# aleju/cat-generator

Measured on AMD Instinct MI355X. Metric: images/sec per G+D step, G32up-c 32x32 RGB bs=128 per GPU, higher is better.
Workload: dtype f32

## Files before the change

cat-generator_amd/csrc/common.h:

```cpp
#pragma once
#include <hip/hip_runtime.h>
#include <algorithm>
#include <stdint.h>
#include <stdio.h>
#include <string.h>
#include "../../include/catgan.h"

namespace cg {

char* err_buf();
int fail(const char* fmt, ...);

inline hipStream_t S(void* s) { return reinterpret_cast<hipStream_t>(s); }

#define CG_HIP(call)                                                              \
    do {                                                                          \
        hipError_t e__ = (call);                                                  \
        if (e__ != hipSuccess)                                                    \
            return cg::fail("%s:%d %s -> %s", __FILE__, __LINE__, #call,          \
                            hipGetErrorString(e__));                              \
    } while (0)

#define CG_LAUNCH_CHECK()                                                         \
    do {                                                                          \
        hipError_t e__ = hipGetLastError();                                       \
        if (e__ != hipSuccess)                                                    \
            return cg::fail("%s:%d kernel launch -> %s", __FILE__, __LINE__,      \
                            hipGetErrorString(e__));                              \
    } while (0)

#define CG_REQUIRE(cond, ...)                                                     \
    do {                                                                          \
        if (!(cond)) return cg::fail(__VA_ARGS__);                                \
    } while (0)

constexpr int kNumCU = 256;

#ifndef CG_TIMING_PROBE
#define CG_TIMING_PROBE 0
#endif
#define CG_PROBE_HALF(fam, T) (((CG_TIMING_PROBE) & (fam)) ? ((T) + 1) / 2 : (T))
constexpr int kEwWgsPerCU = 4, kColReduceWgsPerCU = 1;

enum Opt {
    OPT_SKINNY, OPT_GEMM_BK32, OPT_WINO_BK, OPT_NN_TILE, OPT_TN_TILE, OPT_NN_SPLITS, OPT_TN_SPLITS,
    OPT_XCD_SWIZZLE, OPT_NN_GLDS, OPT_TN_GLDS, OPT_WINO_GLDS, OPT_PAD_SKIP, OPT_WINO3, OPT_WINO_DGRAD_FUSE, OPT_WINO_DGRAD_FUSE_LAUNCHES,
    OPT_WINO3_LAUNCHES, OPT_PACK_WIDE, OPT_SAMPLER_ATOMIC_LAUNCHES, OPT_COUNT
};
long opt(Opt o);
void opt_count(Opt o);

static inline int cdiv(long a, long b) { return (int)((a + b - 1) / b); }

constexpr size_t kColScratchBytes = 8u << 20;
void* col_scratch(hipStream_t stream);
hipStream_t queue_stream(hipStream_t ref, int cls, int slot);
int queue_class(hipStream_t ref, hipStream_t s);

constexpr int MAXG = 4;
constexpr int kMaxStridedGroups = 36;
template <typename T>
__device__ __forceinline__ T sel4(int i, T a, T b, T c, T d) { return i == 0 ? a : (i == 1 ? b : (i == 2 ? c : d)); }
__device__ __forceinline__ float4 ld4(const float* p) { return *reinterpret_cast<const float4*>(p); }
__device__ __forceinline__ float f4c(const float4& v, int i) { return i == 0 ? v.x : (i == 1 ? v.y : (i == 2 ? v.z : v.w)); }
template <typename T>
static inline void set4(T& p0, T& p1, T& p2, T& p3, const T* src, int n) {
    T* const dst[MAXG] = {&p0, &p1, &p2, &p3};
    for (int i = 0; i < MAXG; ++i) *dst[i] = (src && i < n) ? src[i] : nullptr;
}
__device__ __host__ __forceinline__ int phase_map(int a, int d, int pad) { return ((a + d - pad) >> 1) - ((a - pad) >> 1); }
static inline int phase_kp(int k, int pad) { return phase_map(0, k - 1, pad) + 1; }

struct WgradParts {
    const float* part;
    const float* bias_part;
    float* const* gw;
    float* const* gb;
    long gws;
    int ngroups, S, Cin, Cout, kH, kW, pad, ups;
    float scale;
};
int wgrad_finish(hipStream_t st, const WgradParts& w, bool defer);
void wgrad_discard_all();

constexpr int kSkinnyWgradBlocks = 512;
bool skinny_ok(int ngroups, int Cin, int Cout, int kH, int kW, int padH, int padW, int ups);
size_t skinny_wgrad_ws_bytes(int Cin, int Cout);
void skinny_valu_forward(hipStream_t st, const float* x, const float* w, const float* bias, float* y, int N, int H, int W, int Cin, int Cout);
void skinny_valu_wgrad(hipStream_t st, const float* x, const float* dy, float* part, float* bias_part, int N, int H, int W, int Cin, int Cout,
                       int blocks, long ppb);
bool skinny_mfma_ok(int Cin, int Cout, int H, int W);
int skinny_mfma_forward(hipStream_t st, const float* x, const float* w, const float* bias, float* y, int N, int H, int W, int Cin, int Cout);
int skinny_mfma_wgrad(hipStream_t st, const float* x, const float* dy, float* part, float* bias_part, int N, int H, int W, int Cin, int Cout,
                      int max_blocks);

bool head_wgrad_ok(int N, int T, int C, int Co);
int head_wgrad(hipStream_t st, const float* x, const float* dy, float* gw, float* gb, int N, int T, int C, int Co, float scale);
constexpr int kWino3UOffset = 9 * 64 * 64, kWino3UFloats = 16 * 64 * 64;
static inline bool wino3_layer(int Cout, int Cin, int kH, int kW) { return Cout == 64 && Cin == 64 && kH == 3 && kW == 3; }
bool wino3_geom_ok(int ngroups, int N, int H, int W, int Cin, int Cout, int kH, int kW, int padH, int padW, int ups);
int wino3_note_pack(hipStream_t st, int n, const float* const* w, float* const* wf, float* const* wb, const int* Cout, const int* Cin,
                    const int* kH, const int* kW, const int* wb_map);
int wino3_forward(hipStream_t st, int ngroups, const float* const* x, const float* const* wpk, const float* const* bias, float* const* y,
                  int N, int H, int W);

static inline int ew_grid(long n, int per_block = 256) {
    long b = (n + per_block - 1) / per_block;
    if (b < 1) b = 1;
    const long cap = (long)kNumCU * kEwWgsPerCU;
    if (b > cap) b = cap;
    return (int)b;
}

static inline bool al16(const void* p) { return ((uintptr_t)p & 15) == 0; }
template <class... P>
static inline bool vec_ok(long n, const P*... p) { return n % 4 == 0 && (al16(p) && ...); }

constexpr int tile_of_row_c(int l) {
    return ((l < 4 || (l >= 12 && l < 16) || (l >= 20 && l < 28)) ? 0 : 16) +
           ((l < 4 || (l >= 12 && l < 16) || (l >= 20 && l < 28)) ? (l < 4 ? l : (l < 16 ? l - 8 : l - 12)) : (l < 12 ? l - 4 : (l < 20 ? l - 8 : l - 16)));
}
__device__ __forceinline__ int tile_of_row(int l) {
    const bool ga = l < 4 || (l >= 12 && l < 16) || (l >= 20 && l < 28);
    const int rank = ga ? (l < 4 ? l : (l < 16 ? l - 8 : l - 12)) : (l < 12 ? l - 4 : (l < 20 ? l - 8 : l - 16));
    return (ga ? 0 : 16) + rank;
}
__device__ __forceinline__ void wino3_pack_item(const float* __restrict__ w, float* uf, float* ub, int idx) {
    constexpr int C = 64;
    const int co = idx / C, ci = idx % C;
    const float G[4][3] = {{1.f, 0.f, 0.f}, {.5f, .5f, .5f}, {.5f, -.5f, .5f}, {0.f, 0.f, 1.f}};
// ... 233 lines not shown
```

cat-generator_amd/csrc/ops.hip:

```cpp
#include "common.h"
#include <stdarg.h>
#include <stdlib.h>
#include <algorithm>

namespace cg {
char* err_buf() {
    static thread_local char buf[512] = {0};
    return buf;
}
int fail(const char* fmt, ...) {
    va_list ap;
    va_start(ap, fmt);
    vsnprintf(err_buf(), 512, fmt, ap);
    va_end(ap);
    return 1;
}

namespace {
struct OptDef { const char* name; long dflt; };
const OptDef kOptDefs[OPT_COUNT] = {
    {"CG_SKINNY", 1}, {"CG_GEMM_BK32", 1}, {"CG_WINO_BK", 0}, {"CG_NN_TILE", 0}, {"CG_TN_TILE", 0}, {"CG_NN_SPLITS", 0}, {"CG_TN_SPLITS", 0},
    {"CG_XCD_SWIZZLE", 7}, {"CG_NN_GLDS", 1}, {"CG_TN_GLDS", 1}, {"CG_WINO_GLDS", 1}, {"CG_PAD_SKIP", 20}, {"CG_WINO3", 1},
    {"CG_WINO_DGRAD_FUSE", 1}, {"CG_WINO_DGRAD_FUSE_LAUNCHES", 0}, {"CG_WINO3_LAUNCHES", 0}, {"CG_PACK_WIDE", 1},
    {"CG_SAMPLER_ATOMIC_LAUNCHES", 0},
};
long g_opt_val[OPT_COUNT];
int g_opt_state[OPT_COUNT];
}

}
#include <chrono>
#include <mutex>
#include <unordered_map>
#include <vector>
namespace cg {
void* col_scratch(hipStream_t stream) {
    constexpr int kPool = 8, kReserve = 4;
    static std::unordered_map<hipStream_t, void*> blocks;
    static std::vector<void*> pool;
    static std::mutex mu;
    std::lock_guard<std::mutex> lk(mu);
    auto it = blocks.find(stream);
    if (it != blocks.end()) return it->second;
    hipStreamCaptureStatus st = hipStreamCaptureStatusNone;
    const bool capturing = stream && hipStreamIsCapturing(stream, &st) == hipSuccess && st != hipStreamCaptureStatusNone;
    if (capturing && pool.empty()) {
        cg::fail("column reduce: no scratch block left for a stream first used inside a graph capture (run one pass on it before cg_graph_begin)");
        return nullptr;
    }
    if (!capturing && (int)pool.size() <= kReserve) {
        char* p = nullptr;
        hipStreamCaptureMode mode = hipStreamCaptureModeRelaxed;
        (void)hipThreadExchangeStreamCaptureMode(&mode);
        const bool ok = hipMalloc((void**)&p, kColScratchBytes * kPool) == hipSuccess &&
                        hipMemsetAsync(p, 0, kColScratchBytes * kPool, stream) == hipSuccess &&
                        hipStreamSynchronize(stream) == hipSuccess;
        (void)hipThreadExchangeStreamCaptureMode(&mode);
        if (!ok) {
            (void)hipGetLastError();
            if (pool.empty()) { cg::fail("column reduce: cannot allocate %zu bytes of scratch", kColScratchBytes * kPool); return nullptr; }
        } else
            for (int i = kPool - 1; i >= 0; --i) pool.insert(pool.begin(), p + (size_t)i * kColScratchBytes);
    }
    void* blk = pool.back();
    pool.pop_back();
    blocks[stream] = blk;
    return blk;
}
namespace {
__global__ void queue_probe_spin_k(unsigned long long ticks, int* sink) {
    const unsigned long long t0 = wall_clock64();
    while (wall_clock64() - t0 < ticks) { }
    if (ticks == ~0ull) *sink = 1;
}
struct QueuePool {
    std::vector<hipStream_t> s;
    std::unordered_map<hipStream_t, std::vector<int>> cls;
    std::mutex mu;
};
QueuePool& qpool() { static QueuePool p; return p; }
constexpr int kQueuePool = 24;

double probe_pair(hipStream_t a, hipStream_t b, bool both, unsigned long long ticks) {
    (void)hipStreamSynchronize(a);
    if (both) (void)hipStreamSynchronize(b);
    const auto t0 = std::chrono::steady_clock::now();
    hipLaunchKernelGGL(queue_probe_spin_k, dim3(1), dim3(64), 0, a, ticks, (int*)nullptr);
    if (both) hipLaunchKernelGGL(queue_probe_spin_k, dim3(1), dim3(64), 0, b, ticks, (int*)nullptr);
    (void)hipStreamSynchronize(a);
    if (both) (void)hipStreamSynchronize(b);
    return std::chrono::duration<double, std::milli>(std::chrono::steady_clock::now() - t0).count();
}
bool same_queue(hipStream_t a, hipStream_t b) {
    const unsigned long long ticks = 30000;
    int votes = 0;
    for (int r = 0; r < 3; ++r) {
        const double one = probe_pair(a, a, false, ticks), two = probe_pair(a, b, true, ticks);
        if (two > 1.6 * one) ++votes;
    }
    return votes >= 2;
}
}

int queue_classify(hipStream_t ref) {
    QueuePool& p = qpool();
    hipStreamCaptureStatus st = hipStreamCaptureStatusNone;
    if (ref && hipStreamIsCapturing(ref, &st) == hipSuccess && st != hipStreamCaptureStatusNone)
// ... 642 lines not shown
    GRID_STRIDE(i, total) {
        const int c = (int)(i % C);
        long r = i / C;
        const int ox = (int)(r % Wo); r /= Wo;
        const int oy = (int)(r % Ho);
        const long n = r / Ho;
        const long b = ((n * H + 2 * oy) * W + 2 * ox) * C + c;
        const long o01 = C, o10 = (long)W * C, o11 = (long)W * C + C;
        const float v00 = x[b], v01 = x[b + o01], v10 = x[b + o10], v11 = x[b + o11];
        int arg = 0; float m = v00;
        if (v01 > m) { m = v01; arg = 1; }
        if (v10 > m) { m = v10; arg = 2; }
        if (v11 > m) { m = v11; arg = 3; }
        const float g = dy[i];
        dx[b] = arg == 0 ? g : 0.f;
        dx[b + o01] = arg == 1 ? g : 0.f;
        dx[b + o10] = arg == 2 ? g : 0.f;
        dx[b + o11] = arg == 3 ? g : 0.f;
    }
}

template <int VW, bool SPATIAL>
__global__ void mask_mul_k(const float* x, const float* mask, float* y, long n, long HWCV, int CV) {
    typedef Vec<VW> V;
    CG_GRID_STRIDE(i, n) {
        const V m = SPATIAL ? V::ldc(mask, (int)((i / HWCV) * CV + (i % CV))) : V::load(mask, i);
        V v = V::load(x, i);
#pragma unroll
        for (int k = 0; k < VW; ++k) v[k] *= m[k];
        v.store(y, i);
    }
}
using cg::u01;
__global__ void rng_bernoulli_k(float* out, long n, float keep, float value, uint64_t seed, uint64_t offset,
                                const uint64_t* base) {
    if (base) offset += *base;
    GRID_STRIDE(i, n) { out[i] = u01(seed, offset + (uint64_t)i) < keep ? value : 0.f; }
}
__global__ void rng_uniform_k(float* out, long n, float lo, float hi, uint64_t seed, uint64_t offset,
                              const uint64_t* base) {
    if (base) offset += *base;
    GRID_STRIDE(i, n) { out[i] = lo + (hi - lo) * u01(seed, offset + (uint64_t)i); }
}
__global__ void rng_randint_k(int32_t* out, long n, int32_t range, uint64_t seed, uint64_t offset, const uint64_t* base) {
    if (base) offset += *base;
    GRID_STRIDE(i, n) {
        int32_t v = (int32_t)(u01(seed, offset + (uint64_t)i) * (float)range);
        out[i] = v < range ? v : range - 1;
    }
}
__global__ void rng_bernoulli_groups_k(float* out, long n, int G, float keep, float value, uint64_t seed, uint64_t off0,
                                       uint64_t off1, uint64_t off2, uint64_t off3, const uint64_t* base) {
    const uint64_t b = base ? *base : 0ull;
    GRID_STRIDE(i, n * G) {
        const int g = (int)(i / n);
        const uint64_t off = g == 0 ? off0 : (g == 1 ? off1 : (g == 2 ? off2 : off3));
        out[i] = u01(seed, b + off + (uint64_t)(i - (long)g * n)) < keep ? value : 0.f;
    }
}
__global__ void counter_add_k(uint64_t* c, uint64_t d) { if (threadIdx.x == 0 && blockIdx.x == 0) *c += d; }

__global__ void nchw_to_nhwc_k(const float* in, float* out, int N, int C, int H, int W) {
    const long total = (long)N * C * H * W;
    GRID_STRIDE(i, total) {
        const int c = (int)(i % C);
        long r = i / C;
        const int x = (int)(r % W); r /= W;
        const int y = (int)(r % H);
        const long n = r / H;
        out[i] = in[((n * C + c) * H + y) * W + x];
    }
}
__global__ void nhwc_to_nchw_k(const float* in, float* out, int N, int C, int H, int W) {
    const long total = (long)N * C * H * W;
    GRID_STRIDE(i, total) {
        const int x = (int)(i % W);
        long r = i / W;
        const int y = (int)(r % H); r /= H;
        const int c = (int)(r % C);
        const long n = r / C;
        out[i] = in[((n * H + y) * W + x) * C + c];
    }
}
__global__ void copy_channels_k(const float* src, float* dst, long M, int Csrc, int so, int Cdst, int dof, int Cc) {
    const long total = M * Cc;
    GRID_STRIDE(i, total) {
        const int c = (int)(i % Cc);
        const long m = i / Cc;
        dst[m * Cdst + dof + c] = src[m * Csrc + so + c];
    }
}
__global__ void gather_rows_k(const float* src, const int32_t* idx, float* dst, long nrows, long rowlen) {
    const long total = nrows * rowlen;
    GRID_STRIDE(i, total) {
        const long r = i / rowlen, j = i - r * rowlen;
        dst[i] = src[(long)idx[r] * rowlen + j];
    }
}
__global__ void fill_k(float* x, float v, long n) { GRID_STRIDE(i, n) x[i] = v; }
__global__ void axpy_sign_k(float al, const float* x, float* y, long n) {
    GRID_STRIDE(i, n) {
        const float v = x[i];
        y[i] += al * (v > 0.f ? 1.f : (v < 0.f ? -1.f : 0.f));
    }
}
__global__ void scale_k(float* x, float al, long n) { GRID_STRIDE(i, n) x[i] *= al; }
__global__ void clamp_k(float* x, float lo, float hi, long n) {
    GRID_STRIDE(i, n) { x[i] = fminf(fmaxf(x[i], lo), hi); }
}
template <bool SQ>
__global__ void sumred_k(const float* x, long n, double* out) {
    __shared__ double sh[4];
    double s = 0.0;
    GRID_STRIDE(i, n) {
        const float v = x[i];
        s += SQ ? (double)v * (double)v : (double)fabsf(v);
    }
    const double t = block_sum_256(s, sh);
    if (threadIdx.x == 0) atomicAdd(out, t);
}

__global__ void affine_matrix_fwd_k(const float* params, float* T, int N, int ur, int us, int ut) {
    const int P = ur + us + 2 * ut;
    GRID_STRIDE(n, N) {
        const float* p = params + (long)n * P;
        int k = 0;
        float th = 0.f, sc = 1.f, tx = 0.f, ty = 0.f;
        if (ur) th = p[k++];
        if (us) sc = p[k++];
        if (ut) { tx = p[k]; ty = p[k + 1]; }
        const float c = cosf(th), s = sinf(th);
        float* t = T + (long)n * 6;
        t[0] = c * sc;  t[1] = -s * sc; t[2] = c * sc * tx - s * sc * ty;
        t[3] = s * sc;  t[4] = c * sc;  t[5] = s * sc * tx + c * sc * ty;
    }
}
__global__ void affine_matrix_bwd_k(const float* params, const float* gT, float* gparams, int N, int ur, int us, int ut) {
    const int P = ur + us + 2 * ut;
    GRID_STRIDE(n, N) {
        const float* p = params + (long)n * P;
        int k = 0;
        float th = 0.f, sc = 1.f, tx = 0.f, ty = 0.f;
        if (ur) th = p[k++];
        if (us) sc = p[k++];
        if (ut) { tx = p[k]; ty = p[k + 1]; }
        const float c = cosf(th), s = sinf(th);
        const float* g = gT + (long)n * 6;
        float* gp = gparams + (long)n * P;
        k = 0;
        if (ur) {
            const float d0 = -s * sc, d1 = -c * sc, d2 = -s * sc * tx - c * sc * ty;
            const float d3 = c * sc, d4 = -s * sc, d5 = c * sc * tx - s * sc * ty;
            gp[k++] = g[0] * d0 + g[1] * d1 + g[2] * d2 + g[3] * d3 + g[4] * d4 + g[5] * d5;
        }
        if (us) {
            gp[k++] = g[0] * c + g[1] * (-s) + g[2] * (c * tx - s * ty) + g[3] * s + g[4] * c + g[5] * (s * tx + c * ty);
        }
        if (ut) {
            gp[k] = g[2] * (c * sc) + g[5] * (s * sc);
            gp[k + 1] = g[2] * (-s * sc) + g[5] * (c * sc);
        }
    }
}
__global__ void affine_grid_fwd_k(const float* T, float* grid, int N, int H, int W) {
    const long total = (long)N * H * W;
    GRID_STRIDE(i, total) {
// ... 732 lines not shown
    else EW_LAUNCH(bn_bwd_k<1>, total, x, dy, gamma, save_mean, save_invstd, sums, count, total, C, dx);
    EW_LAUNCH(bn_bwd_param_k, (long)C, local_sums, C, ggamma, gbeta, scale);
    return 0;
}

int cg_upsample2x_forward(void* stream, const float* x, float* y, int N, int H, int W, int C) {
    CG_REQUIRE(x && y, "cg_upsample2x_forward: null pointer");
    const long total = (long)N * 4 * H * W * C;
    EW_LAUNCH(ups2_fwd_k, total, x, y, N, H, W, C); return 0;
}
int cg_upsample2x_backward(void* stream, const float* dy, float* dx, int N, int H, int W, int C) {
    CG_REQUIRE(dy && dx, "cg_upsample2x_backward: null pointer");
    const long total = (long)N * H * W * C;
    EW_LAUNCH(ups2_bwd_k, total, dy, dx, N, H, W, C); return 0;
}
int cg_avgpool2_forward(void* stream, const float* x, float* y, int N, int H, int W, int C) {
    CG_REQUIRE(x && y, "cg_avgpool2_forward: null pointer");
    const long total = (long)N * (H / 2) * (W / 2) * C;
    EW_LAUNCH(pool2_fwd_k<false>, total, x, y, N, H, W, C); return 0;
}
int cg_avgpool2_backward(void* stream, const float* dy, float* dx, int N, int H, int W, int C) {
    CG_REQUIRE(dy && dx, "cg_avgpool2_backward: null pointer");
    const long total = (long)N * H * W * C;
    EW_LAUNCH(avgpool2_bwd_k, total, dy, dx, N, H, W, C); return 0;
}
int cg_maxpool2_forward(void* stream, const float* x, float* y, int N, int H, int W, int C) {
    CG_REQUIRE(x && y, "cg_maxpool2_forward: null pointer");
    const long total = (long)N * (H / 2) * (W / 2) * C;
    EW_LAUNCH(pool2_fwd_k<true>, total, x, y, N, H, W, C); return 0;
}
int cg_maxpool2_backward(void* stream, const float* x, const float* dy, float* dx, int N, int H, int W, int C) {
    CG_REQUIRE(x && dy && dx, "cg_maxpool2_backward: null pointer");
    CG_REQUIRE(H % 2 == 0 && W % 2 == 0, "cg_maxpool2_backward: odd spatial size");
    const long total = (long)N * (H / 2) * (W / 2) * C;
    EW_LAUNCH(maxpool2_bwd_k, total, x, dy, dx, N, H, W, C); return 0;
}
int cg_mask_mul(void* stream, const float* x, const float* mask, float* y, int N, long HW, int C, int spatial) {
    CG_REQUIRE(x && mask && y, "cg_mask_mul: null pointer");
    const long total = (long)N * HW * C;
    const bool v4 = spatial ? cg::vec_ok(C, x, y) : cg::vec_ok(total, x, y, mask);
    if (v4 && spatial) EW_LAUNCH((mask_mul_k<4, true>), total / 4, x, mask, y, total / 4, HW * C / 4, C / 4);
    else if (v4) EW_LAUNCH((mask_mul_k<4, false>), total / 4, x, mask, y, total / 4, 0L, 0);
    else if (spatial) EW_LAUNCH((mask_mul_k<1, true>), total, x, mask, y, total, HW * C, C);
    else EW_LAUNCH((mask_mul_k<1, false>), total, x, mask, y, total, 0L, 0);
    return 0;
}
int cg_rng_bernoulli_dev(void* stream, float* out, long n, float keep_prob, float value, uint64_t seed, uint64_t offset,
                         const uint64_t* base) {
    CG_REQUIRE(out, "cg_rng_bernoulli: null pointer");
    EW_LAUNCH(rng_bernoulli_k, n, out, n, keep_prob, value, seed, offset, base); return 0;
}
int cg_rng_bernoulli_dev_grouped(void* stream, float* out, long n_per_group, int ngroups, float keep_prob, float value,
                                 uint64_t seed, uint64_t off0, uint64_t off1, uint64_t off2, uint64_t off3,
                                 const uint64_t* base) {
    CG_REQUIRE(out && ngroups >= 1 && ngroups <= 4, "cg_rng_bernoulli_dev_grouped: bad args");
    EW_LAUNCH(rng_bernoulli_groups_k, n_per_group * ngroups, out, n_per_group, ngroups, keep_prob, value, seed, off0, off1, off2,
              off3, base);
    return 0;
}
int cg_rng_uniform_dev(void* stream, float* out, long n, float lo, float hi, uint64_t seed, uint64_t offset,
                       const uint64_t* base) {
    CG_REQUIRE(out, "cg_rng_uniform: null pointer");
    EW_LAUNCH(rng_uniform_k, n, out, n, lo, hi, seed, offset, base); return 0;
}
int cg_rng_randint_dev(void* stream, int32_t* out, long n, int32_t range, uint64_t seed, uint64_t offset,
                       const uint64_t* base) {
    CG_REQUIRE(out && range > 0, "cg_rng_randint: bad args");
    EW_LAUNCH(rng_randint_k, n, out, n, range, seed, offset, base); return 0;
}
int cg_rng_bernoulli(void* stream, float* out, long n, float keep_prob, float value, uint64_t seed, uint64_t offset) {
    return cg_rng_bernoulli_dev(stream, out, n, keep_prob, value, seed, offset, nullptr);
}
int cg_rng_uniform(void* stream, float* out, long n, float lo, float hi, uint64_t seed, uint64_t offset) {
    return cg_rng_uniform_dev(stream, out, n, lo, hi, seed, offset, nullptr);
}
int cg_rng_randint(void* stream, int32_t* out, long n, int32_t range, uint64_t seed, uint64_t offset) {
    return cg_rng_randint_dev(stream, out, n, range, seed, offset, nullptr);
}
int cg_counter_add(void* stream, uint64_t* counter, uint64_t delta) {
    CG_REQUIRE(counter, "cg_counter_add: null pointer");
    hipLaunchKernelGGL(counter_add_k, dim3(1), dim3(64), 0, cg::S(stream), counter, delta);
    CG_LAUNCH_CHECK(); return 0;
}
int cg_nchw_to_nhwc(void* stream, const float* in, float* out, int N, int C, int H, int W) {
    CG_REQUIRE(in && out, "cg_nchw_to_nhwc: null pointer");
    const long total = (long)N * C * H * W;
    EW_LAUNCH(nchw_to_nhwc_k, total, in, out, N, C, H, W); return 0;
}
int cg_nhwc_to_nchw(void* stream, const float* in, float* out, int N, int C, int H, int W) {
    CG_REQUIRE(in && out, "cg_nhwc_to_nchw: null pointer");
    const long total = (long)N * C * H * W;
    EW_LAUNCH(nhwc_to_nchw_k, total, in, out, N, C, H, W); return 0;
}
int cg_copy_channels(void* stream, const float* src, float* dst, long M, int Csrc, int src_off, int Cdst, int dst_off,
                     int Ccopy) {
    CG_REQUIRE(src && dst, "cg_copy_channels: null pointer");
    CG_REQUIRE(src_off >= 0 && dst_off >= 0 && src_off + Ccopy <= Csrc && dst_off + Ccopy <= Cdst,
               "cg_copy_channels: slice out of range");
    const long total = M * Ccopy;
    EW_LAUNCH(copy_channels_k, total, src, dst, M, Csrc, src_off, Cdst, dst_off, Ccopy); return 0;
}
int cg_gather_rows(void* stream, const float* src, const int32_t* idx, float* dst, long nrows, long rowlen) {
    CG_REQUIRE(src && idx && dst, "cg_gather_rows: null pointer");
    const long total = nrows * rowlen;
    EW_LAUNCH(gather_rows_k, total, src, idx, dst, nrows, rowlen); return 0;
}
int cg_fill(void* stream, float* x, float value, long n) {
    CG_REQUIRE(x, "cg_fill: null pointer");
    EW_LAUNCH(fill_k, n, x, value, n); return 0;
}
int cg_add(void* stream, const float* a, const float* b, float* out, long n) {
    CG_REQUIRE(a && b && out, "cg_add: null pointer");
    if (cg::vec_ok(n, a, b, out)) EW_LAUNCH(add_k<4>, n / 4, a, b, out, n / 4);
    else EW_LAUNCH(add_k<1>, n, a, b, out, n);
    return 0;
}
int cg_axpy(void* stream, float alpha, const float* x, float* y, long n) {
    CG_REQUIRE(x && y, "cg_axpy: null pointer");
    if (cg::vec_ok(n, x, y)) EW_LAUNCH(axpy_k<4>, n / 4, alpha, x, y, n / 4);
    else EW_LAUNCH(axpy_k<1>, n, alpha, x, y, n);
    return 0;
}
int cg_axpy_sign(void* stream, float alpha, const float* x, float* y, long n) {
    CG_REQUIRE(x && y, "cg_axpy_sign: null pointer");
    EW_LAUNCH(axpy_sign_k, n, alpha, x, y, n); return 0;
}
int cg_scale(void* stream, float* x, float alpha, long n) {
    CG_REQUIRE(x, "cg_scale: null pointer");
    EW_LAUNCH(scale_k, n, x, alpha, n); return 0;
}
int cg_clamp(void* stream, float* x, float lo, float hi, long n) {
    CG_REQUIRE(x, "cg_clamp: null pointer");
    EW_LAUNCH(clamp_k, n, x, lo, hi, n); return 0;
}
int cg_sumsq(void* stream, const float* x, long n, double* out) {
    CG_REQUIRE(x && out, "cg_sumsq: null pointer");
    CG_HIP(hipMemsetAsync(out, 0, sizeof(double), cg::S(stream)));
    EW_LAUNCH(sumred_k<true>, n, x, n, out); return 0;
}
int cg_sumabs(void* stream, const float* x, long n, double* out) {
    CG_REQUIRE(x && out, "cg_sumabs: null pointer");
    CG_HIP(hipMemsetAsync(out, 0, sizeof(double), cg::S(stream)));
    EW_LAUNCH(sumred_k<false>, n, x, n, out); return 0;
}

int cg_affine_matrix_forward(void* stream, const float* params, float* T, int N, int use_rot, int use_scale,
                             int use_trans) {
    CG_REQUIRE(params && T, "cg_affine_matrix_forward: null pointer");
    CG_REQUIRE(use_rot || use_scale || use_trans, "cg_affine_matrix_forward: fully parametrised form not supported");
    EW_LAUNCH(affine_matrix_fwd_k, (long)N, params, T, N, use_rot ? 1 : 0, use_scale ? 1 : 0, use_trans ? 1 : 0);
    return 0;
}
int cg_affine_matrix_backward(void* stream, const float* params, const float* gT, float* gparams, int N, int use_rot,
                              int use_scale, int use_trans) {
    CG_REQUIRE(params && gT && gparams, "cg_affine_matrix_backward: null pointer");
    EW_LAUNCH(affine_matrix_bwd_k, (long)N, params, gT, gparams, N, use_rot ? 1 : 0, use_scale ? 1 : 0, use_trans ? 1 : 0);
    return 0;
}
int cg_affine_grid_forward(void* stream, const float* T, float* grid, int N, int H, int W) {
    CG_REQUIRE(T && grid, "cg_affine_grid_forward: null pointer");
    const long total = (long)N * H * W;
    EW_LAUNCH(affine_grid_fwd_k, total, T, grid, N, H, W); return 0;
}
int cg_affine_grid_backward(void* stream, const float* ggrid, float* gT, int N, int H, int W) {
    CG_REQUIRE(ggrid && gT && N > 0, "cg_affine_grid_backward: bad args");
    hipLaunchKernelGGL(affine_grid_bwd_k, dim3(N), dim3(256), 0, cg::S(stream), ggrid, gT, N, H, W);
    CG_LAUNCH_CHECK(); return 0;
}
namespace {
int sampler_forward(void* stream, const float* img, const float* grid, float* out, int N, int Nimg, int Hi, int Wi, int C, int Ho,
                    int Wo) {
    const long total = (long)N * Ho * Wo * C;
    if (cg::vec_ok(C, img, out) && (uintptr_t)grid % 8 == 0) EW_LAUNCH(bilinear_fwd_k<4>, total / 4, img, grid, out, N, Nimg, Hi, Wi, C / 4, Ho, Wo);
// ... 112 lines not shown
```

cat-generator_amd/csrc/wgrad_finish.hip:

```cpp
#include "common.h"
#include <mutex>
#include <unordered_map>
#include <vector>

namespace {

using cg::f4c;
using cg::ld4;
using cg::phase_map;
using cg::sel4;

template <bool UPS, int STEP>
__device__ __forceinline__ float fold(const float* pg, int tap, int ci, int co, int Cin, int Cout, int k, int pad, int kp, long plane, int S,
                                      long sstride, int sp0) {
    float s = 0.f;
    if (UPS) {
        const int dy = tap / k, dx = tap - dy * k;
        for (int sp = sp0; sp < S; sp += STEP)
#pragma unroll
            for (int p = 0; p < 4; ++p) {
                const int tp = phase_map(p >> 1, dy, pad) * kp + phase_map(p & 1, dx, pad);
                s += pg[(long)sp * sstride + (long)p * plane + ((long)tp * Cin + ci) * Cout + co];
            }
    } else {
        const long o = ((long)tap * Cin + ci) * Cout + co;
        constexpr int kInFlight = STEP == 8 ? 4 : 1;
#pragma unroll kInFlight
        for (int sp = sp0; sp < S; sp += STEP) s += pg[(long)sp * sstride + o];
    }
    return s;
}

__device__ __forceinline__ void add4(float4& s, const float4& p) { s.x += p.x; s.y += p.y; s.z += p.z; s.w += p.w; }
template <int STEP>
__device__ __forceinline__ float4 fold4(const float* src, int S, long sstride, int sp0) {
    float4 s = make_float4(0.f, 0.f, 0.f, 0.f);
    int sp = sp0;
    for (; sp + 3 * STEP < S; sp += 4 * STEP) {
        const float4 p0 = ld4(src + (long)sp * sstride), p1 = ld4(src + (long)(sp + STEP) * sstride);
        const float4 p2 = ld4(src + (long)(sp + 2 * STEP) * sstride), p3 = ld4(src + (long)(sp + 3 * STEP) * sstride);
        add4(s, p0); add4(s, p1); add4(s, p2); add4(s, p3);
    }
    for (; sp < S; sp += STEP) add4(s, ld4(src + (long)sp * sstride));
    return s;
}

__device__ __forceinline__ float lane_groups_sum(float (*sh)[33], int ol) {
    float t = 0.f;
#pragma unroll
    for (int r = 0; r < 8; ++r) t += sh[r][ol];
    return t;
}

__device__ __forceinline__ void bias_sum_block(float (*sh)[33], const float* bp, float* gb, int c0, int S, int P, long bsstride, int Cout, float scale) {
    const int cl = threadIdx.x & 31, ln = threadIdx.x >> 5;
    const int c = c0 + cl;
    float s = 0.f;
    if (c < Cout)
        for (int i = ln; i < S * P; i += 8) s += bp[(long)(i / P) * bsstride + (long)(i % P) * Cout + c];
    sh[ln][cl] = s;
    __syncthreads();
    if (ln == 0 && c < Cout) gb[c] += scale * lane_groups_sum(sh, cl);
}

template <bool UPS>
__global__ __launch_bounds__(256) void wgrad_reduce_kernel(const float* part, float* gw, int Cin, int Cout, int k, int KK,
                                                           int pad, int kp, int S, float scale, int CI_T, long sstride) {
    extern __shared__ float sh[];
    const int ci0 = blockIdx.x * CI_T, co0 = blockIdx.y * 32;
    const long plane = (long)(UPS ? kp * kp : KK) * Cin * Cout;
    const int n1 = KK * CI_T * 32;
    for (int idx = threadIdx.x; idx < n1; idx += 256) {
        const int co_l = idx & 31;
        const int r = idx >> 5;
        const int ci_l = r % CI_T, tap = r / CI_T;
        const int ci = ci0 + ci_l, co = co0 + co_l;
        float s = 0.f;
        if (ci < Cin && co < Cout) s = fold<UPS, 1>(part, tap, ci, co, Cin, Cout, k, pad, kp, plane, S, sstride, 0);
        sh[(ci_l * KK + tap) * 33 + co_l] = s;
    }
    __syncthreads();
    const int run = CI_T * KK;
    for (int idx = threadIdx.x; idx < n1; idx += 256) {
        const int j = idx % run, co_l = idx / run;
        const int ci_l = j / KK, tap = j - ci_l * KK;
        const int ci = ci0 + ci_l, co = co0 + co_l;
        if (ci < Cin && co < Cout) {
            float* dst = gw + ((long)co * Cin + ci) * KK + tap;
            *dst += scale * sh[j * 33 + co_l];
        }
    }
}

__global__ __launch_bounds__(256) void bias_part_reduce_kernel(const float* bp, float* gb, int S, int P, long sstride, int Cout, float scale) {
    __shared__ float sh[8][33];
    bias_sum_block(sh, bp, gb, blockIdx.x * 32, S, P, sstride, Cout, scale);
}

struct RedPtrs { float* gw0; float* gw1; float* gw2; float* gw3; float* gb0; float* gb1; float* gb2; float* gb3;
                 long gws; };
struct RedJob {
    const float* part; const float* bias_part;
    RedPtrs rp;
    long sstride, gstride, bsstride;
    int Cin, Cout, k, KK, pad, kp, S, P, ups, ngroups, wblocks, bblocks;
    int block0;
    float scale;
    int tr;
    int v4;
};
constexpr int kRedJobs = 20;
struct RedJobTable { RedJob j[kRedJobs]; int n; };

__device__ __forceinline__ float* gw_of(const RedPtrs& rp, int group) {
    return rp.gws ? rp.gw0 + (long)group * rp.gws : sel4(group, rp.gw0, rp.gw1, rp.gw2, rp.gw3);
}

template <bool UPS>
__device__ __forceinline__ void wgrad_reduce_small(float (*sh)[33], const RedJob& J, int group, int bx) {
    const int ol = threadIdx.x & 31, ln = threadIdx.x >> 5;
    const long total = (long)J.KK * J.Cin * J.Cout, plane = (long)(UPS ? J.kp * J.kp : J.KK) * J.Cin * J.Cout;
    const long i = bx * 32L + ol;
    int co = 0, ci = 0, tap = 0;
    float s = 0.f;
    if (i < total) {
        co = (int)(i % J.Cout);
        const long r = i / J.Cout;
        ci = (int)(r % J.Cin);
        tap = (int)(r / J.Cin);
        s = fold<UPS, 8>(J.part + (long)group * J.gstride, tap, ci, co, J.Cin, J.Cout, J.k, J.pad, J.kp, plane, J.S, J.sstride, ln);
    }
    sh[ln][ol] = s;
    __syncthreads();
    if (ln == 0 && i < total) gw_of(J.rp, group)[((long)co * J.Cin + ci) * J.KK + tap] += J.scale * lane_groups_sum(sh, ol);
}

__device__ __forceinline__ void wgrad_reduce_small_v4(float* shf, const RedJob& J, int group, int bx) {
    float4* sh4 = reinterpret_cast<float4*>(shf);
    const int ol = threadIdx.x & 31, ln = threadIdx.x >> 5;
    const long total = (long)J.KK * J.Cin * J.Cout;
    const long i = bx * 128L + 4 * ol;
    float4 s = make_float4(0.f, 0.f, 0.f, 0.f);
    if (i < total) s = fold4<8>(J.part + (long)group * J.gstride + i, J.S, J.sstride, ln);
    sh4[ln * 32 + ol] = s;
    __syncthreads();
    if (ln < 4 && i < total) {
        float t = 0.f;
#pragma unroll
        for (int r = 0; r < 8; ++r) t += f4c(sh4[r * 32 + ol], ln);
        const long e = i + ln;
        const int co = (int)(e % J.Cout);
        const long rr = e / J.Cout;
        const int ci = (int)(rr % J.Cin), tap = (int)(rr / J.Cin);
        gw_of(J.rp, group)[((long)co * J.Cin + ci) * J.KK + tap] += J.scale * t;
    }
}

__device__ __forceinline__ void wgrad_reduce_t_tile(float (*t)[33], const float* __restrict__ pg, float* __restrict__ gw, int ci0, int co0,
                                                    int Cin, int Cout, int S, long sstride, float scale) {
    const int tx = threadIdx.x & 31, ty = threadIdx.x >> 5;
    if ((Cout & 3) == 0 && (sstride & 3) == 0 && ((uintptr_t)pg & 15) == 0) {
        const int r = threadIdx.x >> 3, c4 = threadIdx.x & 7;
        const float4 s = fold4<1>(pg + (long)(ci0 + r) * Cout + co0 + 4 * c4, S, sstride, 0);
        t[r][4 * c4] = s.x; t[r][4 * c4 + 1] = s.y; t[r][4 * c4 + 2] = s.z; t[r][4 * c4 + 3] = s.w;
    } else
#pragma unroll
    for (int r = ty; r < 32; r += 8) t[r][tx] = fold<false, 1>(pg, 0, ci0 + r, co0 + tx, Cin, Cout, 1, 0, 0, 0, S, sstride, 0);
    __syncthreads();
#pragma unroll
    for (int r = ty; r < 32; r += 8) gw[(long)(co0 + r) * Cin + ci0 + tx] += scale * t[tx][r];
}
__global__ __launch_bounds__(256) void wgrad_reduce_t_kernel(const float* __restrict__ part, float* __restrict__ gw0, long gws, int Cin,
                                                             int Cout, int S, long sstride, long gstride, float scale) {
    __shared__ float t[32][33];
    const int group = blockIdx.z;
    wgrad_reduce_t_tile(t, part + (long)group * gstride, gw0 + (long)group * gws, blockIdx.x * 32, blockIdx.y * 32, Cin, Cout, S, sstride, scale);
}

__device__ __forceinline__ void red_block(float (*sh)[33], const RedJob& J, int group, int bx) {
    if (bx >= J.wblocks) {
        float* gb = sel4(group, J.rp.gb0, J.rp.gb1, J.rp.gb2, J.rp.gb3);
        if (gb) bias_sum_block(sh, J.bias_part + (long)group * J.P * J.Cout, gb, (bx - J.wblocks) * 32, J.S, J.P, J.bsstride, J.Cout, J.scale);
    } else if (J.tr) {
        const int nci = J.Cin / 32;
        wgrad_reduce_t_tile(sh, J.part + (long)group * J.gstride, gw_of(J.rp, group), (bx % nci) * 32, (bx / nci) * 32, J.Cin, J.Cout, J.S, J.sstride, J.scale);
    } else if (J.v4)
        wgrad_reduce_small_v4(&sh[0][0], J, group, bx);
    else if (J.ups)
        wgrad_reduce_small<true>(sh, J, group, bx);
    else
        wgrad_reduce_small<false>(sh, J, group, bx);
}

__global__ __launch_bounds__(256) void wgrad_reduce_small_kernel(RedJob J) {
    __shared__ __attribute__((aligned(16))) float sh[32][33];
    red_block(sh, J, (int)blockIdx.y, (int)blockIdx.x);
}

__global__ __launch_bounds__(256) void wgrad_reduce_batch_kernel(RedJobTable t) {
    __shared__ __attribute__((aligned(16))) float sh[32][33];
    const int b = (int)blockIdx.x;
    int ji = 0;
    for (int q = 1; q < t.n; ++q)
        if (b >= t.j[q].block0) ji = q;
    const RedJob& J = t.j[ji];
    const int per = J.wblocks + J.bblocks;
    const int group = (b - J.block0) / per;
    red_block(sh, J, group, (b - J.block0) - group * per);
}

std::mutex g_red_mu;
std::unordered_map<hipStream_t, std::vector<RedJob>> g_red_queue;

bool transposable(const cg::WgradParts& w) { return w.kH * w.kW == 1 && !w.ups && w.Cin % 32 == 0 && w.Cout % 32 == 0; }

RedJob red_job(const cg::WgradParts& w, bool defer) {
    RedJob job;
    memset(&job, 0, sizeof(job));
    const int nptr = w.gws ? 1 : w.ngroups;
    cg::set4(job.rp.gw0, job.rp.gw1, job.rp.gw2, job.rp.gw3, w.gw, nptr);
    cg::set4(job.rp.gb0, job.rp.gb1, job.rp.gb2, job.rp.gb3, w.gb, nptr);
    job.rp.gws = w.gws;
    job.part = w.part; job.bias_part = w.bias_part;
    job.Cin = w.Cin; job.Cout = w.Cout; job.k = w.kH; job.KK = w.kH * w.kW; job.pad = w.pad; job.ups = w.ups ? 1 : 0;
    job.kp = w.ups ? cg::phase_kp(w.kH, w.pad) : 0;
    job.S = w.S; job.P = w.ups ? 4 : 1; job.ngroups = w.ngroups; job.scale = w.scale;
    const long relems = (long)job.KK * w.Cin * w.Cout;
    job.gstride = (w.ups ? 4L * job.kp * job.kp : job.KK) * w.Cin * w.Cout;
    job.sstride = w.ngroups * job.gstride;
    job.bsstride = (long)w.ngroups * job.P * w.Cout;
    job.wblocks = cg::cdiv(relems, 32); job.bblocks = w.bias_part ? cg::cdiv(w.Cout, 32) : 0;
    if (defer && transposable(w)) {
        job.tr = 1; job.wblocks = (w.Cin / 32) * (w.Cout / 32);
    } else if (!w.ups && w.Cout % 4 == 0 && cg::al16(w.part) && job.sstride % 4 == 0 && job.gstride % 4 == 0) {
        job.v4 = 1; job.wblocks = cg::cdiv(relems, 128);
    }
    return job;
}

int small_reduce(hipStream_t st, bool defer, const RedJob& job) {
    if (defer) {
        std::lock_guard<std::mutex> lk(g_red_mu);
        g_red_queue[st].push_back(job);
        return 0;
    }
    hipLaunchKernelGGL(wgrad_reduce_small_kernel, dim3(job.wblocks + job.bblocks, job.ngroups), dim3(256), 0, st, job);
    CG_LAUNCH_CHECK();
    return 0;
}

}

int cg::wgrad_finish(hipStream_t st, const WgradParts& w, bool defer) {
    const RedJob job = red_job(w, defer);
    const int Cin = w.Cin, Cout = w.Cout, KK = job.KK;
    if (w.gws && transposable(w) && !w.bias_part) {
        hipLaunchKernelGGL(wgrad_reduce_t_kernel, dim3(Cin / 32, Cout / 32, w.ngroups), dim3(256), 0, st, w.part, w.gw[0], w.gws, Cin, Cout, w.S,
                           job.sstride, job.gstride, w.scale);
        CG_LAUNCH_CHECK();
        return 0;
    }
    int ci_t = KK == 1 ? 64 : 8;
    while (ci_t > 1 && (size_t)KK * ci_t * 33 * sizeof(float) > 60000) ci_t >>= 1;
    const size_t shb = (size_t)KK * ci_t * 33 * sizeof(float);
    const dim3 rgrid(cg::cdiv(Cin, ci_t), cg::cdiv(Cout, 32));
    if ((long)rgrid.x * rgrid.y < cg::kNumCU) return small_reduce(st, defer, job);
    for (int gi = 0; gi < w.ngroups; ++gi) {
        const float* pg = w.part + gi * job.gstride;
        float* gwi = w.gws ? w.gw[0] + gi * w.gws : w.gw[gi];
        hipLaunchKernelGGL(w.ups ? wgrad_reduce_kernel<true> : wgrad_reduce_kernel<false>, rgrid, dim3(256), shb, st, pg, gwi, Cin, Cout, w.kH, KK,
                           w.pad, job.kp, w.S, w.scale, ci_t, job.sstride);
        CG_LAUNCH_CHECK();
        if (w.gb && w.gb[gi]) {
            hipLaunchKernelGGL(bias_part_reduce_kernel, dim3(cg::cdiv(Cout, 32)), dim3(256), 0, st, w.bias_part + (long)gi * job.P * Cout, w.gb[gi],
                               w.S, job.P, job.bsstride, Cout, w.scale);
            CG_LAUNCH_CHECK();
        }
    }
    return 0;
}

void cg::wgrad_discard_all() {
    std::lock_guard<std::mutex> lk(g_red_mu);
    for (auto& kv : g_red_queue) kv.second.clear();
}

extern "C" {

int cg_conv2d_wgrad_pending(void* stream, int* njobs) {
    CG_REQUIRE(njobs, "cg_conv2d_wgrad_pending: null pointer");
    std::lock_guard<std::mutex> lk(g_red_mu);
    auto it = g_red_queue.find(cg::S(stream));
    *njobs = it == g_red_queue.end() ? 0 : (int)it->second.size();
    return 0;
}

int cg_conv2d_wgrad_flush(void* stream) {
    hipStream_t st = cg::S(stream);
    std::vector<RedJob> jobs;
    {
        std::lock_guard<std::mutex> lk(g_red_mu);
        auto it = g_red_queue.find(st);
        if (it == g_red_queue.end() || it->second.empty()) return 0;
        jobs.swap(it->second);
    }
    for (size_t j0 = 0; j0 < jobs.size(); j0 += kRedJobs) {
        RedJobTable t;
        memset(&t, 0, sizeof(t));
        t.n = (int)std::min<size_t>(kRedJobs, jobs.size() - j0);
        int blocks = 0;
        for (int q = 0; q < t.n; ++q) {
            t.j[q] = jobs[j0 + q];
            t.j[q].block0 = blocks;
            blocks += t.j[q].ngroups * (t.j[q].wblocks + t.j[q].bblocks);
        }
        hipLaunchKernelGGL(wgrad_reduce_batch_kernel, dim3(blocks), dim3(256), 0, st, t);
        CG_LAUNCH_CHECK();
    }
    return 0;
}

}
```

Baseline: 23610.

## Add wide vectorized wgrad reduce kernel and tiled layout transposes

Adds a wide weight-gradient finish kernel that reads split-K partials as float4 quads, folds upsample phases in registers, fuses the bias reduction into the same launch, and writes back with unrolled batched loads. It also replaces the elementwise NCHW/NHWC conversion kernels with an LDS-tiled transpose when the tiles are well occupied. The aim is fewer launches and more coalesced memory traffic in the reduction and layout passes. The cost is higher register and LDS pressure, and the new code is only used on shapes that pass the alignment checks.

```diff
diff --git a/cat-generator_amd/csrc/common.h b/cat-generator_amd/csrc/common.h
--- a/cat-generator_amd/csrc/common.h
+++ b/cat-generator_amd/csrc/common.h
@@ -45,7 +45,7 @@
 enum Opt {
     OPT_SKINNY, OPT_GEMM_BK32, OPT_WINO_BK, OPT_NN_TILE, OPT_TN_TILE, OPT_NN_SPLITS, OPT_TN_SPLITS,
     OPT_XCD_SWIZZLE, OPT_NN_GLDS, OPT_TN_GLDS, OPT_WINO_GLDS, OPT_PAD_SKIP, OPT_WINO3, OPT_WINO_DGRAD_FUSE, OPT_WINO_DGRAD_FUSE_LAUNCHES,
-    OPT_WINO3_LAUNCHES, OPT_PACK_WIDE, OPT_SAMPLER_ATOMIC_LAUNCHES, OPT_COUNT
+    OPT_WINO3_LAUNCHES, OPT_PACK_WIDE, OPT_SAMPLER_ATOMIC_LAUNCHES, OPT_FINISH_WIDE, OPT_FINISH_WIDE_LAUNCHES, OPT_COUNT
 };
 long opt(Opt o);
 void opt_count(Opt o);
diff --git a/cat-generator_amd/csrc/ops.hip b/cat-generator_amd/csrc/ops.hip
--- a/cat-generator_amd/csrc/ops.hip
+++ b/cat-generator_amd/csrc/ops.hip
@@ -22,7 +22,7 @@
     {"CG_SKINNY", 1}, {"CG_GEMM_BK32", 1}, {"CG_WINO_BK", 0}, {"CG_NN_TILE", 0}, {"CG_TN_TILE", 0}, {"CG_NN_SPLITS", 0}, {"CG_TN_SPLITS", 0},
     {"CG_XCD_SWIZZLE", 7}, {"CG_NN_GLDS", 1}, {"CG_TN_GLDS", 1}, {"CG_WINO_GLDS", 1}, {"CG_PAD_SKIP", 20}, {"CG_WINO3", 1},
     {"CG_WINO_DGRAD_FUSE", 1}, {"CG_WINO_DGRAD_FUSE_LAUNCHES", 0}, {"CG_WINO3_LAUNCHES", 0}, {"CG_PACK_WIDE", 1},
-    {"CG_SAMPLER_ATOMIC_LAUNCHES", 0},
+    {"CG_SAMPLER_ATOMIC_LAUNCHES", 0}, {"CG_FINISH_WIDE", 1}, {"CG_FINISH_WIDE_LAUNCHES", 0},
 };
 long g_opt_val[OPT_COUNT];
 int g_opt_state[OPT_COUNT];
@@ -831,6 +831,27 @@
         out[i] = in[((n * H + y) * W + x) * C + c];
     }
 }
+constexpr int kLayC = 32, kLayP = 16;
+template <int TR, int TC>
+__global__ __launch_bounds__(256) void transpose_tiled_k(const float* in, float* out, int R, int Cc, int tiles_r, int tiles_c, long tiles) {
+    __shared__ float t[TR][TC + 1];
+    for (long tile = blockIdx.x; tile < tiles; tile += gridDim.x) {
+        long b = tile;
+        const int c0 = (int)(b % tiles_c) * TC; b /= tiles_c;
+        const int r0 = (int)(b % tiles_r) * TR;
+        const long base = (b / tiles_r) * R * Cc;
+        for (int idx = threadIdx.x; idx < TR * TC; idx += 256) {
+            const int r = idx / TC, c = idx % TC;
+            if (r0 + r < R && c0 + c < Cc) t[r][c] = in[base + (long)(r0 + r) * Cc + c0 + c];
+        }
+        __syncthreads();
+        for (int idx = threadIdx.x; idx < TR * TC; idx += 256) {
+            const int c = idx / TR, r = idx % TR;
+            if (r0 + r < R && c0 + c < Cc) out[base + (long)(c0 + c) * R + r0 + r] = t[r][c];
+        }
+        __syncthreads();
+    }
+}
 __global__ void copy_channels_k(const float* src, float* dst, long M, int Csrc, int so, int Cdst, int dof, int Cc) {
     const long total = M * Cc;
     GRID_STRIDE(i, total) {
@@ -1729,13 +1750,29 @@
     hipLaunchKernelGGL(counter_add_k, dim3(1), dim3(64), 0, cg::S(stream), counter, delta);
     CG_LAUNCH_CHECK(); return 0;
 }
+static long layout_tiled(int N, int C, int H, int W) {
+    if (cg::opt(cg::OPT_FINISH_WIDE) == 0 || N <= 0 || C <= 0 || H <= 0 || W <= 0) return 0;
+    const long hw = (long)H * W, tc = cg::cdiv(C, kLayC), tp = cg::cdiv(hw, kLayP);
+    const long tiles = N * tc * tp;
+    return 2 * C * hw > tc * kLayC * tp * kLayP ? tiles : 0;
+}
 int cg_nchw_to_nhwc(void* stream, const float* in, float* out, int N, int C, int H, int W) {
     CG_REQUIRE(in && out, "cg_nchw_to_nhwc: null pointer");
+    if (const long tiles = layout_tiled(N, C, H, W)) {
+        hipLaunchKernelGGL((transpose_tiled_k<kLayC, kLayP>), dim3(cg::ew_grid(tiles, 1)), dim3(256), 0, cg::S(stream), in, out, C, H * W,
+                           cg::cdiv(C, kLayC), cg::cdiv((long)H * W, kLayP), tiles);
+        CG_LAUNCH_CHECK(); return 0;
+    }
     const long total = (long)N * C * H * W;
     EW_LAUNCH(nchw_to_nhwc_k, total, in, out, N, C, H, W); return 0;
 }
 int cg_nhwc_to_nchw(void* stream, const float* in, float* out, int N, int C, int H, int W) {
     CG_REQUIRE(in && out, "cg_nhwc_to_nchw: null pointer");
+    if (const long tiles = layout_tiled(N, C, H, W)) {
+        hipLaunchKernelGGL((transpose_tiled_k<kLayP, kLayC>), dim3(cg::ew_grid(tiles, 1)), dim3(256), 0, cg::S(stream), in, out, H * W, C,
+                           cg::cdiv((long)H * W, kLayP), cg::cdiv(C, kLayC), tiles);
+        CG_LAUNCH_CHECK(); return 0;
+    }
     const long total = (long)N * C * H * W;
     EW_LAUNCH(nhwc_to_nchw_k, total, in, out, N, C, H, W); return 0;
 }
diff --git a/cat-generator_amd/csrc/wgrad_finish.hip b/cat-generator_amd/csrc/wgrad_finish.hip
--- a/cat-generator_amd/csrc/wgrad_finish.hip
+++ b/cat-generator_amd/csrc/wgrad_finish.hip
@@ -61,6 +61,27 @@
     sh[ln][cl] = s;
     __syncthreads();
     if (ln == 0 && c < Cout) gb[c] += scale * lane_groups_sum(sh, cl);
+}
+
+template <int U>
+__device__ __forceinline__ void tile_write_back(const float* sh, float* gw, int ci0, int co0, int Cin, int Cout, int KK, int CI_T, int CO_T, float scale) {
+    const int run = CI_T * KK, n1 = run * CO_T;
+    for (int i0 = threadIdx.x; i0 < n1; i0 += 256 * U) {
+        float* dst[U];
+        float g[U], s[U];
+#pragma unroll
+        for (int u = 0; u < U; ++u) {
+            const int idx = i0 + 256 * u;
+            const int j = idx % run, co_l = idx / run;
+            const int ci_l = j / KK, tap = j - ci_l * KK;
+            const int ci = ci0 + ci_l, co = co0 + co_l;
+            dst[u] = idx < n1 && ci < Cin && co < Cout ? gw + ((long)co * Cin + ci) * KK + tap : nullptr;
+            if (dst[u]) { s[u] = sh[j * (CO_T + 1) + co_l]; g[u] = *dst[u]; }
+        }
+#pragma unroll
+        for (int u = 0; u < U; ++u)
+            if (dst[u]) { g[u] += scale * s[u]; *dst[u] = g[u]; }
+    }
 }
 
 template <bool UPS>
@@ -80,16 +101,68 @@
         sh[(ci_l * KK + tap) * 33 + co_l] = s;
     }
     __syncthreads();
-    const int run = CI_T * KK;
-    for (int idx = threadIdx.x; idx < n1; idx += 256) {
-        const int j = idx % run, co_l = idx / run;
-        const int ci_l = j / KK, tap = j - ci_l * KK;
-        const int ci = ci0 + ci_l, co = co0 + co_l;
-        if (ci < Cin && co < Cout) {
-            float* dst = gw + ((long)co * Cin + ci) * KK + tap;
-            *dst += scale * sh[j * 33 + co_l];
-        }
-    }
+    tile_write_back<1>(sh, gw, ci0, co0, Cin, Cout, KK, CI_T, 32, scale);
+}
+
+template <int K>
+__device__ __forceinline__ void wide_quad_sums(float* row, int ld, const float* part, unsigned toff, bool in, long tstride, int KK, int S, long sstride) {
+    if constexpr (K == 0) {
+        for (int tap = 0; tap < KK; ++tap) {
+            const float4 s = in ? fold4<1>(part + tap * tstride + toff, S, sstride, 0) : make_float4(0.f, 0.f, 0.f, 0.f);
+            float* o = row + tap * ld;
+            o[0] = s.x; o[1] = s.y; o[2] = s.z; o[3] = s.w;
+        }
+    } else {
+        constexpr int KP = (K + 1) / 2, PAD = (K - 1) / 2;
+        constexpr int PB = K == 3 ? 4 : 1;
+        float4 acc[K * K];
+#pragma unroll
+        for (int t = 0; t < K * K; ++t) acc[t] = make_float4(0.f, 0.f, 0.f, 0.f);
+        if (in)
+            for (int sp = 0; sp < S; ++sp)
+#pragma unroll
+                for (int p0 = 0; p0 < 4; p0 += PB) {
+                    float4 v[PB][KP * KP];
+#pragma unroll
+                    for (int p = 0; p < PB; ++p)
+#pragma unroll
+                        for (int t = 0; t < KP * KP; ++t) v[p][t] = ld4(part + sp * sstride + ((p0 + p) * KP * KP + t) * tstride + toff);
+#pragma unroll
+                    for (int p = 0; p < PB; ++p)
+#pragma unroll
+                        for (int dy = 0; dy < K; ++dy)
+#pragma unroll
+                            for (int dx = 0; dx < K; ++dx)
+                                add4(acc[dy * K + dx], v[p][phase_map((p0 + p) >> 1, dy, PAD) * KP + phase_map((p0 + p) & 1, dx, PAD)]);
+                }
+#pragma unroll
+        for (int t = 0; t < K * K; ++t) {
+            float* o = row + t * ld;
+            o[0] = acc[t].x; o[1] = acc[t].y; o[2] = acc[t].z; o[3] = acc[t].w;
+        }
+    }
+}
+template <int K>
+__global__ __launch_bounds__(256) __attribute__((amdgpu_waves_per_eu(1, 2))) void wgrad_reduce_wide_kernel(
+    const float* part, float* gw, const float* bias_part, float* gb, int Cin, int Cout, int KK, int S, float scale, int CI_T, int CO_T, long sstride, long bsstride,
+                                                                int nci, int wblocks) {
+    extern __shared__ float sh[];
+    const int b = blockIdx.x;
+    if (b >= wblocks) {
+        bias_sum_block(reinterpret_cast<float(*)[33]>(sh), bias_part, gb, (b - wblocks) * 32, S, K ? 4 : 1, bsstride, Cout, scale);
+        return;
+    }
+    const int ci0 = (b % nci) * CI_T, co0 = (b / nci) * CO_T;
+    const int ld = CO_T + 1, nq = CO_T / 4;
+    const long tstride = (long)Cin * Cout;
+    for (int it = threadIdx.x; it < CI_T * nq; it += 256) {
+        const int q = it % nq, ci_l = it / nq;
+        const int ci = ci0 + ci_l, co = co0 + 4 * q;
+        const bool in = ci < Cin && co < Cout;
+        wide_quad_sums<K>(sh + (long)ci_l * KK * ld + 4 * q, ld, part, (unsigned)ci * Cout + co, in, tstride, KK, S, sstride);
+    }
+    __syncthreads();
+    tile_write_back<9>(sh, gw, ci0, co0, Cin, Cout, KK, CI_T, CO_T, scale);
 }
 
 __global__ __launch_bounds__(256) void bias_part_reduce_kernel(const float* bp, float* gb, int S, int P, long sstride, int Cout, float scale) {
@@ -238,6 +311,26 @@
     return job;
 }
 
+using WideFn = void (*)(const float*, float*, const float*, float*, int, int, int, int, float, int, int, long, long, int, int);
+struct WideShape { WideFn fn; int ci_t, co_t; };
+WideShape wide_shape(const cg::WgradParts& w, const RedJob& job) {
+    WideShape ws{nullptr, 0, 0};
+    const long pick = cg::opt(cg::OPT_FINISH_WIDE);
+    const bool phases_ok = !w.ups || (w.kH == w.kW && (w.kH == 3 || w.kH == 5) && w.pad == (w.kH - 1) / 2);
+    if (pick == 0 || !phases_ok || w.Cout % 4 != 0 || !cg::al16(w.part) || job.sstride % 4 != 0 || job.gstride % 4 != 0 ||
+        (job.gstride / job.P) % 4 != 0 || (long)w.Cin * w.Cout >= (1L << 30))
+        return ws;
+    auto shape = [&](long pk) {
+        ws.ci_t = job.KK == 1 ? 64 : (pk == 2 ? 16 : 8);
+        ws.co_t = pk == 3 ? 64 : 32;
+        while (ws.ci_t > 1 && (size_t)job.KK * ws.ci_t * (ws.co_t + 1) * sizeof(float) > 60000) ws.ci_t >>= 1;
+        return (long)cg::cdiv(w.Cin, ws.ci_t) * cg::cdiv(w.Cout, ws.co_t);
+    };
+    if (shape(pick) < cg::kNumCU) shape(1);
+    ws.fn = !w.ups ? wgrad_reduce_wide_kernel<0> : (w.kH == 3 ? wgrad_reduce_wide_kernel<3> : wgrad_reduce_wide_kernel<5>);
+    return ws;
+}
+
 int small_reduce(hipStream_t st, bool defer, const RedJob& job) {
     if (defer) {
         std::lock_guard<std::mutex> lk(g_red_mu);
@@ -265,9 +358,20 @@
     const size_t shb = (size_t)KK * ci_t * 33 * sizeof(float);
     const dim3 rgrid(cg::cdiv(Cin, ci_t), cg::cdiv(Cout, 32));
     if ((long)rgrid.x * rgrid.y < cg::kNumCU) return small_reduce(st, defer, job);
+    const WideShape ws = wide_shape(w, job);
     for (int gi = 0; gi < w.ngroups; ++gi) {
         const float* pg = w.part + gi * job.gstride;
         float* gwi = w.gws ? w.gw[0] + gi * w.gws : w.gw[gi];
+        if (ws.fn) {
+            float* gbi = w.gb ? w.gb[gi] : nullptr;
+            const int nci = cg::cdiv(Cin, ws.ci_t), wblocks = nci * cg::cdiv(Cout, ws.co_t), bblocks = gbi ? cg::cdiv(Cout, 32) : 0;
+            const size_t wshb = std::max((size_t)KK * ws.ci_t * (ws.co_t + 1), (size_t)8 * 33) * sizeof(float);
+            hipLaunchKernelGGL(ws.fn, dim3(wblocks + bblocks), dim3(256), wshb, st, pg, gwi, gbi ? w.bias_part + (long)gi * job.P * Cout : nullptr,
+                               gbi, Cin, Cout, KK, w.S, w.scale, ws.ci_t, ws.co_t, job.sstride, job.bsstride, nci, wblocks);
+            CG_LAUNCH_CHECK();
+            cg::opt_count(cg::OPT_FINISH_WIDE_LAUNCHES);
+            continue;
+        }
         hipLaunchKernelGGL(w.ups ? wgrad_reduce_kernel<true> : wgrad_reduce_kernel<false>, rgrid, dim3(256), shb, st, pg, gwi, Cin, Cout, w.kH, KK,
                            w.pad, job.kp, w.S, w.scale, ci_t, job.sstride);
         CG_LAUNCH_CHECK();
```

Measured after the change: 23550, median of 2. No clear change (-0.3%).
